# paritybit-ai/XFL

Measured on AMD Instinct MI355X. Metric: 2048-bit Paillier encrypts/s (device-resident), higher is better.
Workload: dtype u32; 1 GPU; DJN private-key (CRT) encrypt, obfuscated, precision 7, 1000000 float64 plaintexts/GPU resident in HBM; key_bits=2048, elements_per_gpu=1000000, fixed_base_window_bits=23, fixed_base_window_split=False, parallelism=shard1, table_bytes=193273528320

## Files before the change

__graft_entry__.py:

```python
import os
import sys

ROOT = os.path.dirname(os.path.abspath(__file__))
if ROOT not in sys.path:
    sys.path.insert(0, ROOT)


def build() -> None:
    from xfl_amd import build as b
    b.build()
    from oracle import build as ob
    ob.build()
    import runpy
    for script in ("build.py", "build_redc_block.py", "build_pmd_ends.py"):
        try:
            runpy.run_path(os.path.join(ROOT, "tests", "native", script), run_name="tests_native_build")["build"]()
        except Exception as exc:
            print(f"warning: device self-test harnesses not built ({script}): {exc}", file=sys.stderr)
    import xfl_amd
    from xfl_amd import _native
    _native.lib()


def smoke() -> None:
    import numpy as np

    from oracle import paillier_oracle as O
    from xfl_amd import _native as nat
    from xfl_amd.paillier.utils import getprimeover
    import random
    import math

    rng = random.Random(7)
    while True:
        p, q = getprimeover(1024, rng=rng), getprimeover(1024, rng=rng)
        if p != q and math.gcd(p - 1, q - 1) == 2:
            break
    n = p * q
    x = rng.getrandbits(n.bit_length()) | (1 << (n.bit_length() - 1))
    h = pow(-(x * x), n, n * n)
    dk = nat.DeviceKey(2048, n, p, q, h, device=0)
    ok = O.derive_private(p, q, h)
    vals = np.random.default_rng(0).standard_normal(64) * 10
    ms = [O.encode_element(ok, float(v), 7)[0] for v in vals]
    rs = [rng.randrange(1, ok["djn_exp_bound"]) for _ in vals]
    ct = nat.words_to_ints(dk.encrypt_words(nat.ints_to_words(ms, dk.nw), nat.ints_to_words(rs, dk.rand_words)))
    want = [O.encrypt_m(ok, m, r) for m, r in zip(ms, rs)]
    assert ct == want, "HIP encrypt differs from the oracle"
    back = nat.words_to_ints(dk.decrypt_words(nat.ints_to_words(ct, dk.n2w)))
    assert back == ms, "HIP decrypt differs from the oracle"
    print("smoke ok: 64 DJN-CRT encryptions + decryptions bit-exact vs oracle on cuda:0")


if __name__ == "__main__":
    build()
    if "--smoke" in sys.argv:
        smoke()
```

xfl_amd/csrc/pdigit_dev.hpp:

```cpp
#pragma once
#include "bn_dev.hpp"

namespace xhe {

struct PmdLdsQ {
  const uint32_t* q;
  XHE_DEV uint4 load4(int i) const { return *reinterpret_cast<const uint4*>(q + (i >> 2) * 256); }
};

template <int K_>
struct PMD {
  static constexpr int K = K_, W = 28, BL = 6;
  static constexpr int NQ = (2 * K + 3) / 4;
  static constexpr uint32_t MASK = (1u << W) - 1u;
  static_assert((K - 1) % BL == 0, "positions 1..K-1 in blocks of 6");
  static_assert((double)(3 * K + 2) * (double)(1ull << 57) < 18446744073709551616.0, "accumulator bound");

  uint32_t p[K];
  uint32_t n0inv;

  XHE_DEV void init(const uint32_t* __restrict__ P, uint32_t ninv) {
#pragma unroll
    for (int j = 0; j < K; ++j) p[j] = __builtin_amdgcn_readfirstlane(P[j]);
    n0inv = ninv;
// ... 223 lines not shown
      "v_mad_u64_u32 %6, vcc, %14, %27, %6\n\t"
      "v_mad_u64_u32 %7, vcc, %14, %28, %7\n\t"
      "v_mad_u64_u32 %8, vcc, %14, %29, %8\n\t"
      "v_mad_u64_u32 %9, vcc, %14, %30, %9\n\t"
      "v_mad_u64_u32 %10, vcc, %14, %31, %10\n\t"
      "v_mad_u64_u32 %11, vcc, %14, %32, %11"
        : "=&v"(T1[j - 1]), "=&v"(T1[j]), "=&v"(T1[j + 1]), "=&v"(T1[j + 2]), "=&v"(T1[j + 3]), "=&v"(T1[j + 4]),
          "=&v"(T2[j - 1]), "=&v"(T2[j]), "=&v"(T2[j + 1]), "=&v"(T2[j + 2]), "=&v"(T2[j + 3]), "=&v"(T2[j + 4])
        : "v"(e), "v"(m1), "v"(m2), "v"(a[j]), "v"(a[j + 1]), "v"(a[j + 2]), "v"(a[j + 3]), "v"(a[j + 4]),
          "v"(a[j + 5]), "v"(c[j]), "v"(c[j + 1]), "v"(c[j + 2]), "v"(c[j + 3]), "v"(c[j + 4]), "v"(c[j + 5]),
          "s"(p[j]), "s"(p[j + 1]), "s"(p[j + 2]), "s"(p[j + 3]), "s"(p[j + 4]), "s"(p[j + 5])
        : "vcc");
  }

  template <bool FIRST = false>
  XHE_DEV void step_row(uint64_t (&T1)[K], uint64_t (&T2)[K], const uint32_t (&a)[K], const uint32_t (&c)[K],
                        uint32_t e, uint32_t en, uint32_t& m1, uint32_t& m2, uint64_t& x1, uint64_t& x2,
                        uint32_t topc) const {
    uint64_t x1n = 0, x2n = 0;
    uint32_t t1 = 0, t2 = 0, m1n = 0, m2n = 0;
    asm("v_mad_u64_u32 %0, vcc, %2, %4, %0\n\t"
        "v_mad_u64_u32 %1, vcc, %3, %4, %1"
        : "+v"(x1), "+v"(x2)
        : "v"(m1), "v"(m2), "s"(p[0])
        : "vcc");
#pragma unroll
    for (int b = 0; b < (K - 1) / BL; ++b) {
      const int j = 1 + BL * b;
      if constexpr (FIRST) blk12_row0(T1, T2, a, c, e, m1, m2, j);
      else blk12_row(T1, T2, a, c, e, m1, m2, j);
      if (b == 0) {
        T1[0] += x1 >> W;
        T2[0] += x2 >> W;
        asm volatile("" : "+v"(T1[0]), "+v"(T2[0]));
      } else if (b == 1) {
        asm("v_mad_u64_u32 %0, vcc, %2, %3, %5\n\t"
            "v_mad_u64_u32 %1, vcc, %2, %4, %6"
            : "=&v"(x1n), "=&v"(x2n)
            : "v"(en), "v"(a[0]), "v"(c[0]), "v"(T1[0]), "v"(T2[0])
            : "vcc");
        asm volatile("" : "+v"(x1n), "+v"(x2n));
      } else if (b == 2) {
        t1 = (uint32_t)x1n * n0inv;
        t2 = (uint32_t)x2n * n0inv;
        asm volatile("" : "+v"(t1), "+v"(t2));
      } else if (b == 3) {
        m1n = t1 & MASK;
        m2n = t2 & MASK;
        asm volatile("" : "+v"(m1n), "+v"(m2n));
      }
      __builtin_amdgcn_sched_barrier(0);
    }
    T1[K - 1] = 0;
    T2[K - 1] = (uint64_t)(topc - m1);
    x1 = x1n;
    x2 = x2n;
    m1 = m1n;
    m2 = m2n;
  }

  XHE_DEV void mul_row(uint32_t (&a)[K], uint32_t (&c)[K], const uint32_t* slot, const uint32_t* topc) const {
    static_assert(K & 1, "the first step alone, then pairs of steps");
    uint64_t T1[K], T2[K];
    uint2 p0 = *reinterpret_cast<const uint2*>(slot);
    uint64_t x1 = mad64(p0.x, a[0], 0ull);
    uint64_t x2 = mad64(p0.x, c[0], 0ull);
    uint32_t m1 = ((uint32_t)x1 * n0inv) & MASK, m2 = ((uint32_t)x2 * n0inv) & MASK;
    step_row<true>(T1, T2, a, c, p0.x, p0.y, m1, m2, x1, x2, topc[0]);
    for (int h = 0; h < K / 2; ++h) {
      const int k = 2 * h + 2;
      const uint32_t tc1 = topc[2 * h + 1], tc2 = topc[2 * h + 2];
      const uint2 p1 = *reinterpret_cast<const uint2*>(slot + (k >> 2) * 256 + (k & 2));
      __builtin_amdgcn_sched_barrier(0);
      step_row(T1, T2, a, c, p0.y, p1.x, m1, m2, x1, x2, tc1);
      __builtin_amdgcn_sched_barrier(0);
      step_row(T1, T2, a, c, p1.x, p1.y, m1, m2, x1, x2, tc2);
      __builtin_amdgcn_sched_barrier(0);
      p0 = p1;
    }
    normalize(T1, a);
    normalize(T2, c);
  }

  static constexpr int EQ = (K + 3) / 4;
  static constexpr int LW = (W * K + 31) / 32;
  static_assert(EQ + (LW + 3) / 4 <= NQ, "e limbs and the log sum share the slot of an interleaved row");

  XHE_DEV static void lam_zero(uint32_t* slot) {
#pragma unroll
    for (int q = 0; q < (LW + 3) / 4; ++q) *reinterpret_cast<uint4*>(slot + (EQ + q) * 256) = make_uint4(0u, 0u, 0u, 0u);
  }
  template <bool FIRST, int NS, int NL>
  XHE_DEV static void add8(uint32_t (&s)[NS], const uint32_t (&l)[NL], int k, uint64_t& cy) {
    if constexpr (FIRST) {
      asm("v_add_co_u32 %0, vcc, %0, %9\n\t"
          "v_addc_co_u32 %1, vcc, %1, %10, vcc\n\t"
          "v_addc_co_u32 %2, vcc, %2, %11, vcc\n\t"
          "v_addc_co_u32 %3, vcc, %3, %12, vcc\n\t"
          "v_addc_co_u32 %4, vcc, %4, %13, vcc\n\t"
          "v_addc_co_u32 %5, vcc, %5, %14, vcc\n\t"
          "v_addc_co_u32 %6, vcc, %6, %15, vcc\n\t"
          "v_addc_co_u32_e64 %7, %8, %7, %16, vcc"
          : "+v"(s[k]), "+v"(s[k + 1]), "+v"(s[k + 2]), "+v"(s[k + 3]), "+v"(s[k + 4]), "+v"(s[k + 5]),
            "+v"(s[k + 6]), "+v"(s[k + 7]), "=s"(cy)
          : "v"(l[k]), "v"(l[k + 1]), "v"(l[k + 2]), "v"(l[k + 3]), "v"(l[k + 4]), "v"(l[k + 5]), "v"(l[k + 6]),
            "v"(l[k + 7])
          : "vcc");
    } else {
      asm("v_addc_co_u32_e64 %0, vcc, %0, %9, %8\n\t"
          "v_addc_co_u32 %1, vcc, %1, %10, vcc\n\t"
          "v_addc_co_u32 %2, vcc, %2, %11, vcc\n\t"
          "v_addc_co_u32 %3, vcc, %3, %12, vcc\n\t"
          "v_addc_co_u32 %4, vcc, %4, %13, vcc\n\t"
          "v_addc_co_u32 %5, vcc, %5, %14, vcc\n\t"
          "v_addc_co_u32 %6, vcc, %6, %15, vcc\n\t"
          "v_addc_co_u32_e64 %7, %8, %7, %16, vcc"
          : "+v"(s[k]), "+v"(s[k + 1]), "+v"(s[k + 2]), "+v"(s[k + 3]), "+v"(s[k + 4]), "+v"(s[k + 5]),
            "+v"(s[k + 6]), "+v"(s[k + 7]), "+s"(cy)
          : "v"(l[k]), "v"(l[k + 1]), "v"(l[k + 2]), "v"(l[k + 3]), "v"(l[k + 4]), "v"(l[k + 5]), "v"(l[k + 6]),
            "v"(l[k + 7])
          : "vcc");
    }
  }
  template <int HW>
  XHE_DEV static void lam_add(uint32_t* slot, const uint32_t (&lam)[HW]) {
    constexpr int LQ = (LW + 3) / 4;
    constexpr int NW = HW < LW ? HW : LW;
    static_assert(HW >= 8 && HW <= 4 * LQ, "at least one block of the chain, at most a whole sum");
    uint32_t s[4 * LQ];
#pragma unroll
    for (int q = 0; q < LQ; ++q) {
      const uint4 v = *reinterpret_cast<const uint4*>(slot + (EQ + q) * 256);
      s[4 * q] = v.x, s[4 * q + 1] = v.y, s[4 * q + 2] = v.z, s[4 * q + 3] = v.w;
    }
    uint64_t cy;
    add8<true>(s, lam, 0, cy);
#pragma unroll
    for (int k = 8; k + 8 <= NW; k += 8) add8<false>(s, lam, k, cy);
#pragma unroll
    for (int k = NW & ~7; k < NW; ++k)
      asm("v_addc_co_u32_e64 %0, %1, %0, %2, %1" : "+v"(s[k]), "+s"(cy) : "v"(lam[k]));
#pragma unroll
    for (int k = NW; k < LW; ++k) asm("v_addc_co_u32_e64 %0, %1, 0, %0, %1" : "+v"(s[k]), "+s"(cy));
#pragma unroll
    for (int q = 0; q < LQ; ++q)
      *reinterpret_cast<uint4*>(slot + (EQ + q) * 256) = make_uint4(s[4 * q], s[4 * q + 1], s[4 * q + 2], s[4 * q + 3]);
  }
  XHE_DEV static void lam_add_slot(uint32_t* slot, const uint32_t* other) {
    constexpr int LQ = (LW + 3) / 4;
    uint32_t o[4 * LQ];
#pragma unroll
    for (int q = 0; q < LQ; ++q) {
      const uint4 v = *reinterpret_cast<const uint4*>(other + (EQ + q) * 256);
      o[4 * q] = v.x, o[4 * q + 1] = v.y, o[4 * q + 2] = v.z, o[4 * q + 3] = v.w;
    }
    lam_add<4 * LQ>(slot, o);
  }

  XHE_DEV static void lam_to_limbs(uint32_t* slot) {
    constexpr int LQ = (LW + 3) / 4;
    uint32_t s[4 * LQ + 1];
#pragma unroll
    for (int q = 0; q < LQ; ++q) {
      const uint4 v = *reinterpret_cast<const uint4*>(slot + (EQ + q) * 256);
      s[4 * q] = v.x, s[4 * q + 1] = v.y, s[4 * q + 2] = v.z, s[4 * q + 3] = v.w;
    }
    s[4 * LQ] = 0u;
    auto limb = [&](int i) -> uint32_t {
      const int bit = W * i, k = bit >> 5, sh = bit & 31;
      return i < K ? (__builtin_amdgcn_alignbit(k + 1 < LW ? s[k + 1] : 0u, s[k], sh) & MASK) : 0u;
    };
#pragma unroll
    for (int q = 0; q < EQ; ++q)
      *reinterpret_cast<uint4*>(slot + q * 256) = make_uint4(limb(4 * q), limb(4 * q + 1), limb(4 * q + 2), limb(4 * q + 3));
  }

  XHE_DEV static void normalize(const uint64_t (&T)[K], uint32_t (&b)[K]) {
    uint64_t cy = 0;
#pragma unroll
    for (int j = 0; j < K; ++j) {
      const uint64_t x = T[j] + cy;
      b[j] = j + 1 < K ? ((uint32_t)x & MASK) : (uint32_t)x;
      cy = x >> W;
      __builtin_amdgcn_sched_barrier(0);
    }
  }

  XHE_DEV void to_mont2(const uint32_t (&a)[K], const uint32_t (&c)[K], uint32_t (&x)[2 * K]) const {
    uint64_t T[2 * K];
#pragma unroll
    for (int j = 0; j < K; ++j) {
      T[j] = 0;
      T[K + j] = a[j];
    }
#pragma unroll
    for (int i = 0; i < K; ++i) {
#pragma unroll
      for (int j = 0; j < K; ++j) T[i + j] = mad64s(c[j], p[i], T[i + j]);
    }
    uint64_t cy = 0;
#pragma unroll
    for (int j = 0; j < 2 * K; ++j) {
      const uint64_t v = T[j] + cy;
      x[j] = j + 1 < 2 * K ? ((uint32_t)v & MASK) : (uint32_t)v;
      cy = v >> W;
    }
  }
};

template <int K>
XHE_DEV void pmd_redc_wide(const PMD<K>& M, uint64_t (&T)[2 * K], uint32_t (&t)[K], uint32_t (&m)[K]) {
  constexpr uint32_t MASK = PMD<K>::MASK;
  uint64_t cy = 0;
#pragma unroll
  for (int i = 0; i < K; ++i) {
    uint64_t x = T[i] + cy;
    const uint32_t mi = ((uint32_t)x * M.n0inv) & MASK;
    m[i] = mi;
    x = mad64s(mi, M.p[0], x);
    cy = x >> 28;
#pragma unroll
    for (int j = 1; j < K; ++j) T[i + j] = mad64s(mi, M.p[j], T[i + j]);
    __builtin_amdgcn_sched_barrier(0);
  }
#pragma unroll
  for (int j = 0; j < K; ++j) {
    const uint64_t x = T[K + j] + cy;
    t[j] = j + 1 < K ? ((uint32_t)x & MASK) : (uint32_t)x;
    cy = x >> 28;
  }
// ... 228 lines not shown
  for (int j = 0; j < K; ++j) {
    const uint32_t v = z[j] + cy;
    z[j] = v & MASK;
    cy = v >> 28;
  }
  pmd_csub<K>(M, z);
  __builtin_amdgcn_sched_barrier(0);
  uint64_t T[2 * K];
#pragma unroll
  for (int j = 0; j < K; ++j) {
    T[j] = u[j];
    T[K + j] = 0;
  }
#pragma unroll
  for (int i = 0; i < K; ++i) {
#pragma unroll
    for (int j = 0; j < K; ++j) T[i + j] = mad64s(z[j], M.p[i], T[i + j]);
  }
  uint64_t c2 = 0;
#pragma unroll
  for (int j = 0; j < 2 * K; ++j) {
    const uint64_t v = T[j] + c2;
    x[j] = (uint32_t)v & MASK;
    c2 = v >> 28;
  }
}

template <int K>
XHE_DEV void pmd_from_mont2(const PMD<K>& M, const uint32_t (&X)[2 * K], const uint32_t* RmodP, uint32_t (&e)[K],
                            uint32_t (&f)[K]) {
  uint32_t m[K];
  {
    uint64_t T[2 * K];
#pragma unroll
    for (int j = 0; j < 2 * K; ++j) T[j] = X[j];
    pmd_redc_wide<K>(M, T, e, m);
  }
  __builtin_amdgcn_sched_barrier(0);
  const bool ge = pmd_csub<K>(M, e);
  __builtin_amdgcn_sched_barrier(0);
  pmd_mod_small<K>(M, m);
  __builtin_amdgcn_sched_barrier(0);
  int64_t br = 0;
#pragma unroll
  for (int j = 0; j < K; ++j) {
    const int64_t v = (int64_t)(ge ? RmodP[j] : 0u) - (int64_t)m[j] + br;
    f[j] = (uint32_t)v & ((1u << 28) - 1u);
    br = v >> 28;
  }
  if (br) {
    int64_t cy = 0;
#pragma unroll
    for (int j = 0; j < K; ++j) {
      const int64_t v = (int64_t)f[j] + (int64_t)M.p[j] + cy;
      f[j] = (uint32_t)v & ((1u << 28) - 1u);
      cy = v >> 28;
    }
  }
}

template <int K, int RW>
XHE_DEV void unpack_pairs_lds(uint32_t* slot) {
  constexpr int HW = RW / 2;
  uint32_t w[RW];
#pragma unroll
  for (int q = 0; q < RW / 4; ++q) {
    const uint4 v = *reinterpret_cast<const uint4*>(slot + q * 256);
    w[4 * q] = v.x;
    w[4 * q + 1] = v.y;
    w[4 * q + 2] = v.z;
    w[4 * q + 3] = v.w;
  }
  auto limb = [&](int base, int i) -> uint32_t {
    const int bit = 28 * i, k = bit >> 5, sh = bit & 31;
    const uint32_t lo = k < HW ? w[base + k] : 0u, hi = k + 1 < HW ? w[base + k + 1] : 0u;
    return i < K ? (__builtin_amdgcn_alignbit(hi, lo, sh) & ((1u << 28) - 1u)) : 0u;
  };
#pragma unroll
  for (int q = 0; q < (2 * K + 3) / 4; ++q)
    *reinterpret_cast<uint4*>(slot + q * 256) =
        make_uint4(limb(0, 2 * q), limb(HW, 2 * q), limb(0, 2 * q + 1), limb(HW, 2 * q + 1));
}

template <int K, int HW>
XHE_DEV void unpack_e_lds(uint32_t* slot) {
  static_assert(HW % 4 == 0 && 32 * HW >= 28 * K - 27, "the packed digit holds K limbs");
  uint32_t w[HW];
#pragma unroll
  for (int q = 0; q < HW / 4; ++q) {
    const uint4 v = *reinterpret_cast<const uint4*>(slot + q * 256);
    w[4 * q] = v.x;
    w[4 * q + 1] = v.y;
    w[4 * q + 2] = v.z;
    w[4 * q + 3] = v.w;
  }
  auto limb = [&](int i) -> uint32_t {
    const int bit = 28 * i, k = bit >> 5, sh = bit & 31;
    const uint32_t lo = k < HW ? w[k] : 0u, hi = k + 1 < HW ? w[k + 1] : 0u;
    return i < K ? (__builtin_amdgcn_alignbit(hi, lo, sh) & ((1u << 28) - 1u)) : 0u;
  };
#pragma unroll
  for (int q = 0; q < (K + 3) / 4; ++q)
    *reinterpret_cast<uint4*>(slot + q * 256) = make_uint4(limb(4 * q), limb(4 * q + 1), limb(4 * q + 2), limb(4 * q + 3));
}

}

namespace xhe {

struct OpLds {
  const uint2* p;
  int stride;
  XHE_DEV uint2 load(int i) const { return p[i * stride]; }
};
struct OpRow {
  const uint2* __restrict__ p;
  XHE_DEV uint2 load(int i) const { return p[i]; }
};

template <int K_, int TPI_>
struct PMDX {
  static constexpr int K = K_, TPI = TPI_, L = K_ / TPI_, W = 27;
  static constexpr uint32_t MASK = (1u << W) - 1u;
  using G = Grp<TPI_>;
  using MN = Mont<K_, 27, TPI_>;
  static_assert(K_ % TPI_ == 0 && L >= 8, "lane groups of at least 8 limbs");
  static_assert((double)K_ * (double)(5ull << 54) < 18446744073709551616.0, "accumulator bound");

  MN M;

  XHE_DEV void init(const uint32_t* N, uint32_t ninv) { M.init(N, ninv); }
  XHE_DEV static bool last() { return G::g() == TPI - 1; }

  template <bool SQ>
  XHE_DEV void blk4(uint64_t (&T1)[L], uint64_t (&T2)[L], const uint32_t (&a)[L], const uint32_t (&c)[L],
                    uint32_t e, uint32_t f, uint32_t m1, uint32_t m2, int j) const {
    if constexpr (SQ) {
      asm("v_mad_u64_u32 %0, vcc, %10, %14, %1\n\t"
          "v_mad_u64_u32 %1, vcc, %10, %15, %2\n\t"
          "v_mad_u64_u32 %2, vcc, %10, %16, %3\n\t"
          "v_mad_u64_u32 %3, vcc, %10, %17, %8\n\t"
          "v_mad_u64_u32 %4, vcc, %11, %18, %5\n\t"
          "v_mad_u64_u32 %5, vcc, %11, %19, %6\n\t"
          "v_mad_u64_u32 %6, vcc, %11, %20, %7\n\t"
          "v_mad_u64_u32 %7, vcc, %11, %21, %9\n\t"
          "v_mad_u64_u32 %0, vcc, %12, %22, %0\n\t"
          "v_mad_u64_u32 %1, vcc, %12, %23, %1\n\t"
          "v_mad_u64_u32 %2, vcc, %12, %24, %2\n\t"
          "v_mad_u64_u32 %3, vcc, %12, %25, %3\n\t"
          "v_mad_u64_u32 %4, vcc, %13, %22, %4\n\t"
          "v_mad_u64_u32 %5, vcc, %13, %23, %5\n\t"
          "v_mad_u64_u32 %6, vcc, %13, %24, %6\n\t"
          "v_mad_u64_u32 %7, vcc, %13, %25, %7"
          : "+v"(T1[j - 1]), "+v"(T1[j]), "+v"(T1[j + 1]), "+v"(T1[j + 2]), "+v"(T2[j - 1]), "+v"(T2[j]),
            "+v"(T2[j + 1]), "+v"(T2[j + 2])
          : "v"(T1[j + 3]), "v"(T2[j + 3]), "v"(e), "v"(f), "v"(m1), "v"(m2), "v"(a[j]), "v"(a[j + 1]),
            "v"(a[j + 2]), "v"(a[j + 3]), "v"(c[j]), "v"(c[j + 1]), "v"(c[j + 2]), "v"(c[j + 3]), "v"(M.nl[j]),
            "v"(M.nl[j + 1]), "v"(M.nl[j + 2]), "v"(M.nl[j + 3])
          : "vcc");
    } else {
      asm("v_mad_u64_u32 %0, vcc, %10, %14, %1\n\t"
          "v_mad_u64_u32 %1, vcc, %10, %15, %2\n\t"
          "v_mad_u64_u32 %2, vcc, %10, %16, %3\n\t"
          "v_mad_u64_u32 %3, vcc, %10, %17, %8\n\t"
          "v_mad_u64_u32 %4, vcc, %10, %18, %5\n\t"
          "v_mad_u64_u32 %5, vcc, %10, %19, %6\n\t"
          "v_mad_u64_u32 %6, vcc, %10, %20, %7\n\t"
          "v_mad_u64_u32 %7, vcc, %10, %21, %9\n\t"
          "v_mad_u64_u32 %4, vcc, %11, %14, %4\n\t"
          "v_mad_u64_u32 %5, vcc, %11, %15, %5\n\t"
          "v_mad_u64_u32 %6, vcc, %11, %16, %6\n\t"
          "v_mad_u64_u32 %7, vcc, %11, %17, %7\n\t"
          "v_mad_u64_u32 %0, vcc, %12, %22, %0\n\t"
          "v_mad_u64_u32 %1, vcc, %12, %23, %1\n\t"
          "v_mad_u64_u32 %2, vcc, %12, %24, %2\n\t"
          "v_mad_u64_u32 %3, vcc, %12, %25, %3\n\t"
          "v_mad_u64_u32 %4, vcc, %13, %22, %4\n\t"
          "v_mad_u64_u32 %5, vcc, %13, %23, %5\n\t"
          "v_mad_u64_u32 %6, vcc, %13, %24, %6\n\t"
          "v_mad_u64_u32 %7, vcc, %13, %25, %7"
          : "+v"(T1[j - 1]), "+v"(T1[j]), "+v"(T1[j + 1]), "+v"(T1[j + 2]), "+v"(T2[j - 1]), "+v"(T2[j]),
            "+v"(T2[j + 1]), "+v"(T2[j + 2])
          : "v"(T1[j + 3]), "v"(T2[j + 3]), "v"(e), "v"(f), "v"(m1), "v"(m2), "v"(a[j]), "v"(a[j + 1]),
            "v"(a[j + 2]), "v"(a[j + 3]), "v"(c[j]), "v"(c[j + 1]), "v"(c[j + 2]), "v"(c[j + 3]), "v"(M.nl[j]),
            "v"(M.nl[j + 1]), "v"(M.nl[j + 2]), "v"(M.nl[j + 3])
          : "vcc");
// ... 522 lines not shown
```

xfl_amd/csrc/xhe_kernels.hpp:

```cpp
#pragma once
#include "bn_dev.hpp"
#include "keydev.hpp"
#include "pdigit_dev.hpp"

#include <type_traits>

namespace xhe {

enum : int32_t { ST_OK = 0, ST_OVERFLOW = 1, ST_VALUE = 2 };

struct EncVal {
  int32_t st, e;
  int neg, w;
  uint32_t v0, v1, v2;
};

XHE_DEV EncVal encode_value(double v, int mode, int e0, int has_max, int max_exp) {
  EncVal r{ST_OK, 0, 0, 0, 0u, 0u, 0u};
  uint64_t bits = __double_as_longlong(v);
  r.neg = (int)(bits >> 63);
  int bexp = (int)((bits >> 52) & 0x7FF);
  uint64_t frac = bits & ((1ull << 52) - 1);
  int e;
  if (mode == 0) {
// ... 445 lines not shown
  SqLds<MP2>(img).put(b);
  M.load_words(b, m_words + (size_t)e * key.nw, key.nw);
  M.mul(b, ARow{nR});
  b[0] += 1u;
  M.mul(b, ALdsQ{mine});
  M.reduce_once(b);
  M.store_strided(b, ws + (size_t)prime * 2 * MP2::S4 * count + e, (int)count);
}

template <class MP2, int RW>
__global__ void __launch_bounds__(128, 2) k_djn_pow_lds(KeyDev key, const uint32_t* __restrict__ Np2,
                                                        const uint32_t* __restrict__ Nq2,
                                                        const uint32_t* __restrict__ m_words,
                                                        const uint32_t* __restrict__ a_words, int aw, int64_t count,
                                                        uint32_t* __restrict__ ws) {
  static_assert(MP2::TPI == 1, "LDS row staging is per lane");
  __shared__ __attribute__((aligned(16))) uint32_t img_all[2][(MP2::S4 / 4) * 256];
  const int64_t e = (int64_t)blockIdx.x * blockDim.x + threadIdx.x;
  const int prime = blockIdx.y;
  uint32_t* img = img_all[(threadIdx.x >> 6) & 1];
  if (e >= count) return;
  djn_prime_lds<MP2, RW>(key, prime ? Nq2 : Np2, prime ? key.q2 : key.p2, prime ? key.tab_q2 : key.tab_p2,
                     prime ? key.nR2_q2 : key.nR2_p2, prime ? key.nR_q2 : key.nR_p2, m_words, a_words, aw, count, e,
                     prime, img, img + (threadIdx.x & 63) * 4, ws);
}

template <class MP2, int KP, int RW, int G = 1>
__global__ void __launch_bounds__(128, 2) k_djn_pmd(KeyDev key, const uint32_t* __restrict__ Pp,
                                                    const uint32_t* __restrict__ Pq,
                                                    const uint32_t* __restrict__ m_words,
                                                    const uint32_t* __restrict__ a_words, int aw, int64_t count,
                                                    uint32_t* __restrict__ ws) {
  static_assert(MP2::TPI == 1 && MP2::S == 2 * KP && MP2::W == 28, "digits of the one-lane P^2 shape");
  using D = PMD<KP>;
  constexpr int NQ = D::NQ > MP2::S4 / 4 ? D::NQ : MP2::S4 / 4;
  __shared__ __attribute__((aligned(16))) uint32_t img_all[2][NQ * 256];
  __shared__ __attribute__((aligned(16))) uint32_t topc[(KP + 3) & ~3];
  const int prime = blockIdx.y;
  const uint32_t* tc = prime ? key.topc_q : key.topc_p;
  if (threadIdx.x < KP) topc[threadIdx.x] = tc[threadIdx.x];
  __syncthreads();
  static_assert(G >= 1 && G <= 64 && (G & (G - 1)) == 0, "lane groups of a power of two, inside one wave");
  const int64_t t = (int64_t)blockIdx.x * blockDim.x + threadIdx.x;
  const int64_t e = t / G;
  const int g = (int)(threadIdx.x & (G - 1));
  if (e >= count) return;
  uint32_t* img = img_all[(threadIdx.x >> 6) & 1];
  uint32_t* slot = img + (threadIdx.x & 63) * 4;
  const uint32_t* tab = prime ? key.tab_q2 : key.tab_p2;
  const uint32_t* ae = a_words + (size_t)e * aw;
  D M;
  M.init(prime ? Pq : Pp, prime ? key.q.n0inv : key.p.n0inv);
  auto stage = [&](int w) XHE_INL {
    int64_t row0;
    const uint32_t d = win_digit(key, ae, aw, w, row0);
    const uint32_t* row = tab + (size_t)(row0 + d) * key.tab_rs;
#pragma unroll
    for (int k = 0; k < RW / 8; ++k)
      __builtin_amdgcn_global_load_lds((xhe_glb_void*)(row + 4 * k), (xhe_lds_void*)(img + k * 256), 16, 0, 0);
    uint32_t lam[RW / 2];
#pragma unroll
    for (int k = 0; k < RW / 8; ++k) {
      const uint4 v = *reinterpret_cast<const uint4*>(row + RW / 2 + 4 * k);
      lam[4 * k] = v.x, lam[4 * k + 1] = v.y, lam[4 * k + 2] = v.z, lam[4 * k + 3] = v.w;
    }
    asm volatile("s_waitcnt vmcnt(0)" ::: "memory");
    D::template lam_add<RW / 2>(slot, lam);
    unpack_e_lds<KP, RW / 2>(slot);
  };
  if (G == 1 || g == 0) {
    const uint32_t* mw = m_words + (size_t)e * key.nw;
    uint32_t sw[4];
    bool neg;
    const bool is_short = pmd_short_classify<KP>(mw, key.nw, key.n_words, sw, neg);
    if (__builtin_amdgcn_ballot_w64(!is_short) == 0ull)
      pmd_lam_short<KP>(M, slot, sw, neg, prime ? key.ms_q : key.ms_p);
    else
      pmd_lam_plain<KP>(M, slot, mw, key.nw, prime ? key.mu_q : key.mu_p, prime ? Pq : Pp);
  } else {
    D::lam_zero(slot);
  }
  __builtin_amdgcn_sched_barrier(0);
  uint32_t a[KP], c[KP];
  if (G == 1 || g < key.nwin) {
    stage(g);
#pragma unroll
    for (int q = 0; q < D::EQ; ++q) {
      const uint4 v = *reinterpret_cast<const uint4*>(slot + q * 256);
      if (4 * q < KP) a[4 * q] = v.x;
      if (4 * q + 1 < KP) a[4 * q + 1] = v.y;
      if (4 * q + 2 < KP) a[4 * q + 2] = v.z;
      if (4 * q + 3 < KP) a[4 * q + 3] = v.w;
    }
#pragma unroll
    for (int j = 0; j < KP; ++j) c[j] = 0u;
  }
  for (int w = g + G; w < key.nwin; w += G) {
    stage(w);
    M.mul_row(a, c, slot, topc);
  }
  if constexpr (G > 1) {
#pragma unroll
    for (int s = 1; s < G; s <<= 1) {
      const bool writer = (g & (2 * s - 1)) == s && g < key.nwin;
      const bool reader = (g & (2 * s - 1)) == 0 && g + s < key.nwin;
      if (reader) D::lam_add_slot(slot, slot + 4 * s);
      wave_sync_mem_();
      if (writer) {
#pragma unroll
        for (int q = 0; q < D::NQ; ++q)
          *reinterpret_cast<uint4*>(slot + q * 256) =
              make_uint4(2 * q < KP ? a[2 * q] : 0u, 2 * q < KP ? c[2 * q] : 0u, 2 * q + 1 < KP ? a[2 * q + 1] : 0u,
                         2 * q + 1 < KP ? c[2 * q + 1] : 0u);
      }
      wave_sync_mem_();
      if (reader) M.mul(a, c, slot + 4 * s, topc);
      wave_sync_mem_();
    }
    if (g != 0) return;
  }
  uint32_t b[MP2::L];
  pmd_exit<KP>(M, a, c, slot, topc, prime ? Pq : Pp, b);
  __builtin_amdgcn_sched_barrier(0);
  MP2 N;
  const int64_t eo = ((int64_t)blockIdx.x * blockDim.x + (uint32_t)opaque_i((int)threadIdx.x)) / G;
  N.store_strided(b, ws + (size_t)prime * 2 * MP2::S4 * count + eo, (int)count);
}

template <int KP>
XHE_DEV void pmd_pow_uniform(const PMD<KP>& M, uint32_t (&a)[KP], uint32_t (&c)[KP], const uint32_t* ex, int ebits,
                             uint4* __restrict__ tab_base, int lane, int G, uint32_t* slot, const uint32_t* topc) {
  constexpr int NQ = PMD<KP>::NQ;
#define tab (tab_base + opaque_i(lane))
  auto quad = [&](int q) -> uint4 {
    return make_uint4(2 * q < KP ? a[2 * q] : 0u, 2 * q < KP ? c[2 * q] : 0u, 2 * q + 1 < KP ? a[2 * q + 1] : 0u,
                      2 * q + 1 < KP ? c[2 * q + 1] : 0u);
  };
  auto put_slot = [&]() XHE_INL {
#pragma unroll
    for (int q = 0; q < NQ; ++q) *reinterpret_cast<uint4*>(slot + q * 256) = quad(q);
  };
  auto put_tab = [&](int t) XHE_INL {
#pragma unroll
    for (int q = 0; q < NQ; ++q) tab[((size_t)t * NQ + q) * G] = quad(q);
  };
  auto tab_to_slot = [&](int t) XHE_INL {
    uint4 v[NQ];
#pragma unroll
    for (int q = 0; q < NQ; ++q) v[q] = tab[((size_t)t * NQ + q) * G];
#pragma unroll
    for (int q = 0; q < NQ; ++q) *reinterpret_cast<uint4*>(slot + q * 256) = v[q];
  };
  auto tab_to_regs = [&](int t) XHE_INL {
#pragma unroll
    for (int q = 0; q < NQ; ++q) {
      const uint4 v = tab[((size_t)t * NQ + q) * G];
      if (2 * q < KP) a[2 * q] = v.x, c[2 * q] = v.y;
      if (2 * q + 1 < KP) a[2 * q + 1] = v.z, c[2 * q + 1] = v.w;
    }
  };
  auto bit = [&](int i) { return (ex[i >> 5] >> (i & 31)) & 1u; };
  int i = ebits - 1;
  while (i >= 0 && !bit(i)) --i;
  int pend_sq = 0, pend_mul = -1;
  bool sq = false;
  auto next_op = [&]() -> bool {
    while (true) {
      if (pend_sq > 0) {
        put_slot();
        --pend_sq;
        sq = true;
        return true;
      }
      if (pend_mul >= 0) {
        tab_to_slot(pend_mul);
        pend_mul = -1;
        sq = false;
        return true;
      }
      if (i < 0) return false;
      if (!bit(i)) {
        pend_sq = 1;
        --i;
      } else {
        int j = i - 4 < 0 ? 0 : i - 4;
        while (!bit(j)) ++j;
        uint32_t val = 0;
        for (int k = i; k >= j; --k) val = (val << 1) | bit(k);
        pend_sq = i - j + 1;
        pend_mul = (int)(val >> 1);
        i = j - 1;
      }
    }
  };
  put_tab(0);
  put_slot();
  sq = true;
  int t = -1;
#pragma unroll 1
  while (true) {
    if (sq) M.sqr(a, c, slot, topc);
    else M.mul(a, c, slot, topc);
// ... 1938 lines not shown
```

Baseline: 48.83 million encrypts/s.

## Pair fixed-base window products before accumulation and batch log-sum loads

```diff
diff --git a/__graft_entry__.py b/__graft_entry__.py
--- a/__graft_entry__.py
+++ b/__graft_entry__.py
@@ -12,7 +12,7 @@
     from oracle import build as ob
     ob.build()
     import runpy
-    for script in ("build.py", "build_redc_block.py", "build_pmd_ends.py"):
+    for script in ("build.py", "build_redc_block.py", "build_pmd_ends.py", "build_pmd_pair.py"):
         try:
             runpy.run_path(os.path.join(ROOT, "tests", "native", script), run_name="tests_native_build")["build"]()
         except Exception as exc:
diff --git a/xfl_amd/csrc/pdigit_dev.hpp b/xfl_amd/csrc/pdigit_dev.hpp
--- a/xfl_amd/csrc/pdigit_dev.hpp
+++ b/xfl_amd/csrc/pdigit_dev.hpp
@@ -329,6 +329,105 @@
     normalize(T2, c);
   }
 
+  XHE_DEV void blk6(uint64_t (&T)[K], const uint32_t (&r)[K], uint32_t e, uint32_t m, int j) const {
+    asm(
+      "v_mad_u64_u32 %0, vcc, %7, %9, %1\n\t"
+      "v_mad_u64_u32 %1, vcc, %7, %10, %2\n\t"
+      "v_mad_u64_u32 %2, vcc, %7, %11, %3\n\t"
+      "v_mad_u64_u32 %3, vcc, %7, %12, %4\n\t"
+      "v_mad_u64_u32 %4, vcc, %7, %13, %5\n\t"
+      "v_mad_u64_u32 %5, vcc, %7, %14, %6\n\t"
+      "v_mad_u64_u32 %0, vcc, %8, %15, %0\n\t"
+      "v_mad_u64_u32 %1, vcc, %8, %16, %1\n\t"
+      "v_mad_u64_u32 %2, vcc, %8, %17, %2\n\t"
+      "v_mad_u64_u32 %3, vcc, %8, %18, %3\n\t"
+      "v_mad_u64_u32 %4, vcc, %8, %19, %4\n\t"
+      "v_mad_u64_u32 %5, vcc, %8, %20, %5"
+        : "+v"(T[j - 1]), "+v"(T[j]), "+v"(T[j + 1]), "+v"(T[j + 2]), "+v"(T[j + 3]), "+v"(T[j + 4])
+        : "v"(T[j + 5]), "v"(e), "v"(m), "v"(r[j]), "v"(r[j + 1]), "v"(r[j + 2]), "v"(r[j + 3]), "v"(r[j + 4]),
+          "v"(r[j + 5]), "s"(p[j]), "s"(p[j + 1]), "s"(p[j + 2]), "s"(p[j + 3]), "s"(p[j + 4]), "s"(p[j + 5])
+        : "vcc");
+  }
+  XHE_DEV void blk6_0(uint64_t (&T)[K], const uint32_t (&r)[K], uint32_t e, uint32_t m, int j) const {
+    asm(
+      "v_mad_u64_u32 %0, vcc, %6, %8, 0\n\t"
+      "v_mad_u64_u32 %1, vcc, %6, %9, 0\n\t"
+      "v_mad_u64_u32 %2, vcc, %6, %10, 0\n\t"
+      "v_mad_u64_u32 %3, vcc, %6, %11, 0\n\t"
+      "v_mad_u64_u32 %4, vcc, %6, %12, 0\n\t"
+      "v_mad_u64_u32 %5, vcc, %6, %13, 0\n\t"
+      "v_mad_u64_u32 %0, vcc, %7, %14, %0\n\t"
+      "v_mad_u64_u32 %1, vcc, %7, %15, %1\n\t"
+      "v_mad_u64_u32 %2, vcc, %7, %16, %2\n\t"
+      "v_mad_u64_u32 %3, vcc, %7, %17, %3\n\t"
+      "v_mad_u64_u32 %4, vcc, %7, %18, %4\n\t"
+      "v_mad_u64_u32 %5, vcc, %7, %19, %5"
+        : "=&v"(T[j - 1]), "=&v"(T[j]), "=&v"(T[j + 1]), "=&v"(T[j + 2]), "=&v"(T[j + 3]), "=&v"(T[j + 4])
+        : "v"(e), "v"(m), "v"(r[j]), "v"(r[j + 1]), "v"(r[j + 2]), "v"(r[j + 3]), "v"(r[j + 4]), "v"(r[j + 5]),
+          "s"(p[j]), "s"(p[j + 1]), "s"(p[j + 2]), "s"(p[j + 3]), "s"(p[j + 4]), "s"(p[j + 5])
+        : "vcc");
+  }
+
+  template <bool FIRST = false>
+  XHE_DEV void step_one(uint64_t (&T)[K], const uint32_t (&r)[K], uint32_t e, uint32_t en, uint32_t& m,
+                        uint64_t& x) const {
+    uint64_t xn = 0;
+    uint32_t t = 0, mn = 0;
+    asm("v_mad_u64_u32 %0, vcc, %1, %2, %0" : "+v"(x) : "v"(m), "s"(p[0]) : "vcc");
+#pragma unroll
+    for (int b = 0; b < (K - 1) / BL; ++b) {
+      const int j = 1 + BL * b;
+      if constexpr (FIRST) blk6_0(T, r, e, m, j);
+      else blk6(T, r, e, m, j);
+      if (b == 0) {
+        T[0] += x >> W;
+        asm volatile("" : "+v"(T[0]));
+      } else if (b == 1) {
+        asm("v_mad_u64_u32 %0, vcc, %1, %2, %3" : "=&v"(xn) : "v"(en), "v"(r[0]), "v"(T[0]) : "vcc");
+        asm volatile("" : "+v"(xn));
+      } else if (b == 2) {
+        t = (uint32_t)xn * n0inv;
+        asm volatile("" : "+v"(t));
+      } else if (b == 3) {
+        mn = t & MASK;
+        asm volatile("" : "+v"(mn));
+      }
+      __builtin_amdgcn_sched_barrier(0);
+    }
+    T[K - 1] = 0;
+    x = xn;
+    m = mn;
+  }
+
+  static constexpr int PQ = NQ - (K + 3) / 4;
+  XHE_DEV void mul_pair(uint32_t (&r)[K], uint32_t* slot, const uint32_t* topc) const {
+    static_assert(K & 1, "the first step alone, then pairs of steps");
+    static_assert(PQ >= 0 && K / 2 - 1 <= 2 * PQ - 1, "c12 is written over e2 limbs already read");
+    const uint32_t* es = slot + PQ * 256;
+    uint64_t T[K];
+    uint2 p0 = *reinterpret_cast<const uint2*>(es);
+    uint64_t x = mad64(p0.x, r[0], 0ull);
+    uint32_t m = ((uint32_t)x * n0inv) & MASK;
+    slot[1] = topc[0] - m;
+    step_one<true>(T, r, p0.x, p0.y, m, x);
+    for (int h = 0; h < K / 2; ++h) {
+      const int k = 2 * h + 2;
+      const uint32_t tc1 = topc[2 * h + 1], tc2 = topc[2 * h + 2];
+      const uint2 p1 = *reinterpret_cast<const uint2*>(es + (k >> 2) * 256 + (k & 2));
+      __builtin_amdgcn_sched_barrier(0);
+      slot[h * 256 + 3] = tc1 - m;
+      step_one(T, r, p0.y, p1.x, m, x);
+      __builtin_amdgcn_sched_barrier(0);
+      slot[(h + 1) * 256 + 1] = tc2 - m;
+      step_one(T, r, p1.x, p1.y, m, x);
+      __builtin_amdgcn_sched_barrier(0);
+      p0 = p1;
+    }
+    normalize(T, r);
+#pragma unroll
+    for (int j = 0; j < K; ++j) slot[(j >> 1) * 256 + 2 * (j & 1)] = r[j];
+  }
+
   static constexpr int EQ = (K + 3) / 4;
   static constexpr int LW = (W * K + 31) / 32;
   static_assert(EQ + (LW + 3) / 4 <= NQ, "e limbs and the log sum share the slot of an interleaved row");
@@ -393,6 +492,20 @@
     for (int q = 0; q < LQ; ++q)
       *reinterpret_cast<uint4*>(slot + (EQ + q) * 256) = make_uint4(s[4 * q], s[4 * q + 1], s[4 * q + 2], s[4 * q + 3]);
   }
+  template <int HW>
+  XHE_DEV static void lam_acc(uint32_t (&s)[4 * ((LW + 3) / 4)], const uint32_t (&lam)[HW]) {
+    constexpr int NW = HW < LW ? HW : LW;
+    static_assert(HW >= 8 && HW <= 4 * ((LW + 3) / 4), "at least one block of the chain, at most a whole sum");
+    uint64_t cy;
+    add8<true>(s, lam, 0, cy);
+#pragma unroll
+    for (int k = 8; k + 8 <= NW; k += 8) add8<false>(s, lam, k, cy);
+#pragma unroll
+    for (int k = NW & ~7; k < NW; ++k)
+      asm("v_addc_co_u32_e64 %0, %1, %0, %2, %1" : "+v"(s[k]), "+s"(cy) : "v"(lam[k]));
+#pragma unroll
+    for (int k = NW; k < LW; ++k) asm("v_addc_co_u32_e64 %0, %1, 0, %0, %1" : "+v"(s[k]), "+s"(cy));
+  }
   XHE_DEV static void lam_add_slot(uint32_t* slot, const uint32_t* other) {
     constexpr int LQ = (LW + 3) / 4;
     uint32_t o[4 * LQ];
@@ -787,7 +900,7 @@
         make_uint4(limb(0, 2 * q), limb(HW, 2 * q), limb(0, 2 * q + 1), limb(HW, 2 * q + 1));
 }
 
-template <int K, int HW>
+template <int K, int HW, int QO = 0>
 XHE_DEV void unpack_e_lds(uint32_t* slot) {
   static_assert(HW % 4 == 0 && 32 * HW >= 28 * K - 27, "the packed digit holds K limbs");
   uint32_t w[HW];
@@ -806,7 +919,41 @@
   };
 #pragma unroll
   for (int q = 0; q < (K + 3) / 4; ++q)
-    *reinterpret_cast<uint4*>(slot + q * 256) = make_uint4(limb(4 * q), limb(4 * q + 1), limb(4 * q + 2), limb(4 * q + 3));
+    *reinterpret_cast<uint4*>(slot + (QO + q) * 256) =
+        make_uint4(limb(4 * q), limb(4 * q + 1), limb(4 * q + 2), limb(4 * q + 3));
+}
+
+template <int K, int HW>
+XHE_DEV void unpack_e0_lds(uint32_t* slot) {
+  static_assert(HW % 4 == 0 && 32 * HW >= 28 * K - 27, "the packed digit holds K limbs");
+  uint32_t w[HW];
+#pragma unroll
+  for (int q = 0; q < HW / 4; ++q) {
+    const uint4 v = *reinterpret_cast<const uint4*>(slot + q * 256);
+    w[4 * q] = v.x;
+    w[4 * q + 1] = v.y;
+    w[4 * q + 2] = v.z;
+    w[4 * q + 3] = v.w;
+  }
+  auto limb = [&](int i) -> uint32_t {
+    const int bit = 28 * i, k = bit >> 5, sh = bit & 31;
+    const uint32_t lo = k < HW ? w[k] : 0u, hi = k + 1 < HW ? w[k + 1] : 0u;
+    return i < K ? (__builtin_amdgcn_alignbit(hi, lo, sh) & ((1u << 28) - 1u)) : 0u;
+  };
+#pragma unroll
+  for (int q = 0; q < (2 * K + 3) / 4; ++q)
+    *reinterpret_cast<uint4*>(slot + q * 256) = make_uint4(limb(2 * q), 0u, limb(2 * q + 1), 0u);
+}
+
+template <int K, int HW>
+XHE_DEV void unpack_e_regs(const uint32_t (&w)[HW], uint32_t (&r)[K]) {
+  static_assert(32 * HW >= 28 * K - 27, "the packed digit holds K limbs");
+#pragma unroll
+  for (int i = 0; i < K; ++i) {
+    const int bit = 28 * i, k = bit >> 5, sh = bit & 31;
+    const uint32_t lo = k < HW ? w[k] : 0u, hi = k + 1 < HW ? w[k + 1] : 0u;
+    r[i] = __builtin_amdgcn_alignbit(hi, lo, sh) & ((1u << 28) - 1u);
+  }
 }
 
 }
diff --git a/xfl_amd/csrc/xhe_kernels.hpp b/xfl_amd/csrc/xhe_kernels.hpp
--- a/xfl_amd/csrc/xhe_kernels.hpp
+++ b/xfl_amd/csrc/xhe_kernels.hpp
@@ -551,6 +551,109 @@
   }
   __builtin_amdgcn_sched_barrier(0);
   uint32_t a[KP], c[KP];
+  if constexpr (G == 1) {
+    constexpr int LQ = (D::LW + 3) / 4, HW = RW / 2;
+    {
+      uint32_t s[4 * LQ];
+#pragma unroll
+      for (int q = 0; q < LQ; ++q) {
+        const uint4 v = *reinterpret_cast<const uint4*>(slot + (D::EQ + q) * 256);
+        s[4 * q] = v.x, s[4 * q + 1] = v.y, s[4 * q + 2] = v.z, s[4 * q + 3] = v.w;
+      }
+      auto lam_row = [&](int w, uint32_t (&lam)[HW]) XHE_INL {
+        int64_t row0;
+        const uint32_t d = win_digit(key, ae, aw, w, row0);
+        const uint32_t* row = tab + (size_t)(row0 + d) * key.tab_rs;
+#pragma unroll
+        for (int k = 0; k < HW / 4; ++k) {
+          const uint4 v = *reinterpret_cast<const uint4*>(row + HW + 4 * k);
+          lam[4 * k] = v.x, lam[4 * k + 1] = v.y, lam[4 * k + 2] = v.z, lam[4 * k + 3] = v.w;
+        }
+      };
+      int w = 0;
+      for (; w + 4 <= key.nwin; w += 4) {
+        uint32_t l0[HW], l1[HW], l2[HW], l3[HW];
+        lam_row(w, l0);
+        lam_row(w + 1, l1);
+        lam_row(w + 2, l2);
+        lam_row(w + 3, l3);
+        D::template lam_acc<HW>(s, l0);
+        D::template lam_acc<HW>(s, l1);
+        D::template lam_acc<HW>(s, l2);
+        D::template lam_acc<HW>(s, l3);
+      }
+      for (; w < key.nwin; ++w) {
+        uint32_t l0[HW];
+        lam_row(w, l0);
+        D::template lam_acc<HW>(s, l0);
+      }
+      uint32_t* park = ws + (size_t)prime * 2 * MP2::S4 * count + e;
+#pragma unroll
+      for (int k = 0; k < D::LW; ++k) park[(size_t)k * count] = s[k];
+    }
+    __builtin_amdgcn_sched_barrier(0);
+    auto ae_now = [&]() XHE_INL -> const uint32_t* {
+      return a_words + (size_t)((int64_t)blockIdx.x * blockDim.x + (uint32_t)opaque_i((int)threadIdx.x)) * aw;
+    };
+    auto dma_e = [&](int w) XHE_INL {
+      int64_t row0;
+      const uint32_t d = win_digit(key, ae_now(), aw, w, row0);
+      const uint32_t* row = tab + (size_t)(row0 + d) * key.tab_rs;
+#pragma unroll
+      for (int k = 0; k < RW / 8; ++k)
+        __builtin_amdgcn_global_load_lds((xhe_glb_void*)(row + 4 * k), (xhe_lds_void*)(img + k * 256), 16, 0, 0);
+    };
+    dma_e(0);
+    asm volatile("s_waitcnt vmcnt(0)" ::: "memory");
+    unpack_e_lds<KP, HW>(slot);
+#pragma unroll
+    for (int q = 0; q < D::EQ; ++q) {
+      const uint4 v = *reinterpret_cast<const uint4*>(slot + q * 256);
+      if (4 * q < KP) a[4 * q] = v.x;
+      if (4 * q + 1 < KP) a[4 * q + 1] = v.y;
+      if (4 * q + 2 < KP) a[4 * q + 2] = v.z;
+      if (4 * q + 3 < KP) a[4 * q + 3] = v.w;
+    }
+#pragma unroll
+    for (int j = 0; j < KP; ++j) c[j] = 0u;
+    for (int w = 1; w < key.nwin; w += 2) {
+      if (w + 1 < key.nwin) {
+        uint32_t r[KP];
+        dma_e(w + 1);
+        int64_t row0;
+        const uint32_t d = win_digit(key, ae_now(), aw, w, row0);
+        const uint32_t* row = tab + (size_t)(row0 + d) * key.tab_rs;
+        uint32_t pw[HW];
+#pragma unroll
+        for (int k = 0; k < HW / 4; ++k) {
+          const uint4 v = *reinterpret_cast<const uint4*>(row + 4 * k);
+          pw[4 * k] = v.x, pw[4 * k + 1] = v.y, pw[4 * k + 2] = v.z, pw[4 * k + 3] = v.w;
+        }
+        asm volatile("s_waitcnt vmcnt(0)" ::: "memory");
+        unpack_e_lds<KP, HW, D::PQ>(slot);
+        unpack_e_regs<KP, HW>(pw, r);
+        __builtin_amdgcn_sched_barrier(0);
+        M.mul_pair(r, slot, topc);
+      } else {
+        dma_e(w);
+        asm volatile("s_waitcnt vmcnt(0)" ::: "memory");
+        unpack_e0_lds<KP, HW>(slot);
+      }
+      __builtin_amdgcn_sched_barrier(0);
+      M.mul(a, c, slot, topc);
+    }
+    {
+      const int64_t ep = (int64_t)blockIdx.x * blockDim.x + (uint32_t)opaque_i((int)threadIdx.x);
+      const uint32_t* park = ws + (size_t)prime * 2 * MP2::S4 * count + ep;
+      uint32_t s[4 * LQ];
+#pragma unroll
+      for (int k = 0; k < 4 * LQ; ++k) s[k] = k < D::LW ? park[(size_t)k * count] : 0u;
+#pragma unroll
+      for (int q = 0; q < LQ; ++q)
+        *reinterpret_cast<uint4*>(slot + (D::EQ + q) * 256) = make_uint4(s[4 * q], s[4 * q + 1], s[4 * q + 2], s[4 * q + 3]);
+    }
+    __builtin_amdgcn_sched_barrier(0);
+  } else {
   if (G == 1 || g < key.nwin) {
     stage(g);
 #pragma unroll
@@ -587,6 +690,7 @@
       wave_sync_mem_();
     }
     if (g != 0) return;
+  }
   }
   uint32_t b[MP2::L];
   pmd_exit<KP>(M, a, c, slot, topc, prime ? Pq : Pp, b);
```

New measurement: 51.19 million encrypts/s, median of 6. 1.05x the previous value.
